# line/Human-Interaction-Generation

Measured on AMD Instinct MI355X. Metric: denoiser-fwd frames/s @ B=64·T=196, higher is better.
Workload: dtype f32; 1 GPU; MotionTransformer forward incl. the per-call cross-attention text side, BASELINE config 2: B=64/GPU T=196 F=150 d=512 L=8 H=8 ff=1024 N=77 Lt=256, linear attention, text embeddings supplied (CLIP stubbed); parallelism=dp1

## Files before the change

human-interaction-generation_amd/csrc/denoiser.hip:

```cpp
#include <stdarg.h>
#include <stdio.h>
#include <string.h>

#include "hig_common.h"
#include "hig_host.h"

static thread_local char g_err[512] = "";
int hig_set_error(int code, const char* fmt, ...) {
  va_list ap;
  va_start(ap, fmt);
  vsnprintf(g_err, sizeof(g_err), fmt, ap);
  va_end(ap);
  return code;
}
extern "C" int hig_last_error(char* buf, int n) {
  if (buf && n > 0) {
    strncpy(buf, g_err, (size_t)n - 1);
    buf[n - 1] = 0;
  }
  return (int)strlen(g_err);
}
extern "C" int hig_version(void) { return 100; }

namespace {
// ... 416 lines not shown
  }
  return &s;
}

thread_local hig_denoiser_plan_t g_last_schedule = {-1};
hig_denoiser_call call_of(int entry, const Dims& D, bool training, bool has_xf_out, int facts, bool capturing) {
  return {entry, D.B, D.T, D.F, D.d, D.E, D.ff, D.L, D.H, D.hd, D.N, D.nsty, D.two, D.full, D.prec, training,
          has_xf_out || entry == HIG_DN_ENTRY_TEXT32 || entry == HIG_DN_ENTRY_TEXT16, facts, capturing};
}
hig_denoiser_plan_t plan_entry(int entry, const Dims& D, bool training, bool has_xf_out, int facts, hipStream_t st, SideStream** side) {
  const hig_denoiser_call c = call_of(entry, D, training, has_xf_out, facts, is_capturing(st));
  hig_denoiser_plan_t p = hig_denoiser_plan_for(c, hig_denoiser_switch_values(), hig_chip_cus(), hig_gemm_wsp32_active());
  SideStream* s = side_streams(p.wants_side_stream, c.capturing);
  if (!s) p.text_fork = p.split = p.fork_emb = p.fork_text = p.wgrad_fork = 0;
  if (side) *side = s;
  g_last_schedule = p;
  return p;
}

struct ThirdStreamJoin {
  hipStream_t s3 = nullptr, st = nullptr;
  hipEvent_t ev = nullptr;
  bool armed = false;
  void arm(hipStream_t s3_, hipEvent_t ev_, hipStream_t st_) { s3 = s3_; ev = ev_; st = st_; armed = true; }
  ~ThirdStreamJoin() {
    if (!armed) return;
    (void)hipEventRecord(ev, s3);
    (void)hipStreamWaitEvent(st, ev, 0);
  }
};

}

static int denoiser_fwd_impl(const hig_dims* dims, const void* const* params, const void* const* derived32, const float* x, const int64_t* t,
                             const int64_t* length, const float* xf_proj, const float* xf_out_for_text, const void* textctx, float* out,
                             void* workspace, int training, hig_stream_t stream);
extern "C" int hig_denoiser_fwd(const hig_dims* dims, const void* const* params, const float* x,
                                const int64_t* t, const int64_t* length, const float* xf_proj,
                                const void* textctx, float* out, void* workspace, int training,
                                hig_stream_t stream) {
  return denoiser_fwd_impl(dims, params, nullptr, x, t, length, xf_proj, nullptr, textctx, out, workspace, training, stream);
}
extern "C" int hig_denoiser_fwd_text(const hig_dims* dims, const void* const* params, const float* x, const int64_t* t,
                                     const int64_t* length, const float* xf_proj, const float* xf_out, void* textctx, float* out,
                                     void* workspace, int training, hig_stream_t stream) {
  HIG_REQUIRE(xf_out, "hig_denoiser_fwd_text: null argument");
  return denoiser_fwd_impl(dims, params, nullptr, x, t, length, xf_proj, xf_out, textctx, out, workspace, training, stream);
}
extern "C" int hig_denoiser_fwd_x(const hig_dims* dims, const void* const* params, const void* const* derived32, const float* x,
                                  const int64_t* t, const int64_t* length, const float* xf_proj, const float* xf_out, void* textctx,
                                  float* out, void* workspace, int training, hig_stream_t stream) {
  return denoiser_fwd_impl(dims, params, derived32, x, t, length, xf_proj, xf_out, textctx, out, workspace, training, stream);
}
static int denoiser_fwd_impl(const hig_dims* dims, const void* const* params, const void* const* derived32, const float* x, const int64_t* t,
                             const int64_t* length, const float* xf_proj, const float* xf_out_for_text, const void* textctx, float* out,
                             void* workspace, int training, hig_stream_t stream) {
  Dims D;
  HIG_TRY(check_dims(dims, D));
  HIG_REQUIRE(params && x && t && xf_proj && textctx && out && workspace, "hig_denoiser_fwd: null argument");
  HIG_REQUIRE(!D.bf16, "hig_denoiser_fwd: bf16 storage goes through hig_denoiser_fwd_bf16");
  const FwdLayout w = fwd_layout(D, training);
  const TextLayout tl = text_layout(D, training);
  float* ws = static_cast<float*>(workspace);
  const float* tc = static_cast<const float*>(textctx);
  hipStream_t st = hig_stream(stream);
  const int d = D.d, E = D.E;
  const int64_t M = D.M;
  const int64_t ss_ld = (int64_t)D.nsty * D.L * 2 * d;
  const int Bp = D.B / 2;

  HIG_TRY(hig_zero_async(ws + w.gtail, HIG_GEMM_TAIL_CNT_BYTES, st));
  const TailScratchScope tail_scope(ws + w.gtail);

  SideStream* side = nullptr;
  const hig_denoiser_plan_t plan = plan_entry(HIG_DN_ENTRY_FWD32, D, training, xf_out_for_text != nullptr,
                                              derived_facts(derived32_table(D, derived32), HIG_D32_TEXT_KV_W), st, &side);
  hipEvent_t* text_ev = nullptr;
  ThirdStreamJoin text_join;
  if (xf_out_for_text) {
    if (plan.text_fork) {
      HIG_TRY(hig_zero_async(ws + w.gtail3, HIG_GEMM_TAIL_CNT_BYTES, st));
      if (hipEventRecord(side->ready, st) != hipSuccess || hipStreamWaitEvent(side->s3, side->ready, 0) != hipSuccess)
        return hig_set_error(HIG_EHIP, "text fork failed");
      hig_gemm_set_tail_scratch(ws + w.gtail3, HIG_GEMM_TAIL_BYTES);
      const int rc = text_context_impl(D, params, derived32, xf_out_for_text, const_cast<void*>(textctx), training, plan.text_batched, side->s3,
                                       side->text_done);
      hig_gemm_set_tail_scratch(ws + w.gtail, HIG_GEMM_TAIL_BYTES);
      text_join.arm(side->s3, side->text_done[0], st);
      if (rc != HIG_OK) return rc;
      text_ev = side->text_done;
    } else {
      HIG_TRY(text_context_impl(D, params, derived32, xf_out_for_text, const_cast<void*>(textctx), training, plan.text_batched, st, nullptr));
    }
  }
  HIG_TRY(hig_timestep_embedding(t, D.B, d, ws + w.te, stream));
  float* few_scratch = ws + w.layer0;
  const int64_t few_floats = w.total - w.layer0;
  HIG_TRY(hig_gemm_few_rows(G(ws + w.te, d, 0, P(params, HIG_P_TE0_W), d, 0, ws + w.te_h, E, D.B, E, d)
                                .epi(HIG_EPI_BIAS, P(params, HIG_P_TE0_B)).prec(D.prec).g, few_scratch, few_floats, st));
  HIG_TRY(hig_gemm_few_rows(G(ws + w.te_h, E, 0, P(params, HIG_P_TE2_W), E, 0, ws + w.emb, E, D.B, E, E)
                                .silu(0).epi(HIG_EPI_BIAS_RES, P(params, HIG_P_TE2_B)).res(xf_proj, E).prec(D.prec).g,
                            few_scratch, few_floats, st));
  HIG_TRY(hig_gemm_few_rows(G(ws + w.emb, E, 0, P(params, HIG_P_STY_EMB_W), E, 0, ws + w.ss, ss_ld, D.B, ss_ld, E)
                                .silu(0).epi(HIG_EPI_BIAS, P(params, HIG_P_STY_EMB_B)).prec(D.prec).g, few_scratch, few_floats,
                            st));
  {
    G ge(x, D.F, 0, P(params, HIG_P_JOINT_W), D.F, 0, ws + w.h0, d, M, d, D.F);
    ge.epi(HIG_EPI_BIAS_POS, P(params, HIG_P_JOINT_B)).pos(P(params, HIG_P_SEQ_EMB), d, D.T).prec(D.prec);
    ge.g.pos_shift = D.two ? 1 : 0;
    HIG_TRY(hig_gemm_launch(ge.g, 1, nullptr, st));
  }
  const int64_t* len_partner = nullptr;
  if (D.two) {
    HIG_TRY(hig_gemm_launch(G(x, (int64_t)D.T * D.F, 0, P(params, HIG_P_JOINT2_W), 4, 0, ws + w.h0, (int64_t)D.T * d,
                              D.B, d, 4).epi(HIG_EPI_BIAS, P(params, HIG_P_JOINT2_B)).g, 1, nullptr, st));
    int64_t* lp = reinterpret_cast<int64_t*>(ws + w.lenp);
    hipLaunchKernelGGL(swap_halves_i64_kernel, dim3((D.B + 255) / 256), dim3(256), 0, st, length, D.B, (int64_t)D.T, lp);
    HIG_CHECK_LAUNCH();
    len_partner = lp;
  }
  const bool fuse_apply = plan.fuse_apply, fold32 = plan.fold32;
  const Derived d32 = derived32_table(D, derived32);
  int layer_rc = HIG_OK;
  auto layer = [&](int l, const float* hin_full, int b0, int nb, hipStream_t s, float* cscr) -> const float* {
    hig_stream_t hs = reinterpret_cast<hig_stream_t>(s);
    float* lb = ws + w.layer0 + w.lstride * l;
    const int64_t r0 = (int64_t)b0 * D.T, Mh = (int64_t)nb * D.T;
    const int64_t aoff = (int64_t)b0 * D.H * D.hd * D.hd;
    const float* ssl = ws + w.ss + (int64_t)(D.nsty * l) * 2 * d + (int64_t)b0 * ss_ld;
    const float* ss_ffn = ssl + (int64_t)(D.nsty - 1) * 2 * d;
    const int64_t* len = length ? length + b0 : nullptr;
    const float* hin = hin_full + r0 * d;
    auto R = [&](int64_t off, int64_t ld) { return lb + off + r0 * ld; };
    auto fail = [&](int rc) -> const float* { layer_rc = rc; return nullptr; };
#define HIG_L(expr) do { const int rc_ = (expr); if (rc_ != HIG_OK) return fail(rc_); } while (0)
    const int np = d >> 6;
    float* lnst = ws + w.lnstats + r0 * np * 2;
    auto folded = [&](int k) { return fold32 && d32.layer(l, HIG_D32_SA_QKV_W + 3 * k) != nullptr; };
// ... 1085 lines not shown
  for (int l = 0; l < D.L; ++l) {
    char* lb = base + tl.layer0 + tl.lstride * l;
    HIG_TRY(hig_ln_bf16(xf_out, 1, D.Lt, D.Mt, D.Lt, PL(params, l, HIG_L_CA_TNORM_W), PL(params, l, HIG_L_CA_TNORM_B), nullptr, 0, 0, 0,
                        lb + tl.xfn, D.Lt, stream));
    HIG_TRY(hig_gemm16_launch(G16(lb + tl.xfn, D.Lt, PL16(params16, l, HIG_L_CA_KV_W), D.Lt, lb + tl.kv, 2 * D.d, D.Mt, 2 * D.d, D.Lt)
                                  .epi(HIG_EPI_BIAS, PL(params, l, HIG_L_CA_KV_B)).g, st));
    HIG_TRY(ctx16(D, plan.ctx_mm16, lb + tl.kv, lb + tl.kv + (int64_t)D.d * 2, 2 * D.d, D.B, D.N, nullptr, reinterpret_cast<float*>(lb + tl.Ac),
                  reinterpret_cast<float*>(lb + tl.kstc), reinterpret_cast<float*>(base + tl.cscr), lb + tl.Atc, stream));
  }
  return HIG_OK;
}

extern "C" int hig_denoiser_fwd_bf16_train(const hig_dims* dims, const void* const* params, const void* const* params16,
                                           const float* x, const int64_t* t, const int64_t* length, const float* xf_proj,
                                           const void* textctx, float* out, void* workspace, hig_stream_t stream) {
  Dims D;
  HIG_TRY(check_dims(dims, D));
  HIG_TRY(require_bf16_train(D, "hig_denoiser_fwd_bf16_train"));
  HIG_REQUIRE(params && params16 && x && t && xf_proj && textctx && out && workspace, "hig_denoiser_fwd_bf16_train: null argument");
  const Fwd16TLayout w = fwd16t_layout(D);
  const Text16TLayout tl = text16t_layout(D);
  char* ws = static_cast<char*>(workspace);
  const char* tc = static_cast<const char*>(textctx);
  hipStream_t st = hig_stream(stream);
  const hig_denoiser_plan_t plan = plan_entry(HIG_DN_ENTRY_FWD16_TRAIN, D, true, false, 0, st);
  const int d = D.d, E = D.E;
  const int64_t M = D.M;
  const int64_t ss_ld = (int64_t)D.nsty * D.L * 2 * d;
  float* te = reinterpret_cast<float*>(ws + w.te);
  float* te_h = reinterpret_cast<float*>(ws + w.te_h);
  float* emb = reinterpret_cast<float*>(ws + w.emb);
  float* ss = reinterpret_cast<float*>(ws + w.ss);
  float* few = reinterpret_cast<float*>(ws + w.few);
  const int64_t few_floats = w.few_bytes / 4;
  HIG_TRY(hig_timestep_embedding(t, D.B, d, te, stream));
  HIG_TRY(hig_gemm_few_rows(G(te, d, 0, P(params, HIG_P_TE0_W), d, 0, te_h, E, D.B, E, d).epi(HIG_EPI_BIAS, P(params, HIG_P_TE0_B)).g,
                            few, few_floats, st));
  HIG_TRY(hig_gemm_few_rows(G(te_h, E, 0, P(params, HIG_P_TE2_W), E, 0, emb, E, D.B, E, E).silu(0)
                                .epi(HIG_EPI_BIAS_RES, P(params, HIG_P_TE2_B)).res(xf_proj, E).g, few, few_floats, st));
  HIG_TRY(hig_gemm_few_rows(G(emb, E, 0, P(params, HIG_P_STY_EMB_W), E, 0, ss, ss_ld, D.B, ss_ld, E).silu(0)
                                .epi(HIG_EPI_BIAS, P(params, HIG_P_STY_EMB_B)).g, few, few_floats, st));
  if (d % 128 == 0 && D.F <= 512) {
    HIG_TRY(hig_joint_embed_bf16(x, M, D.F, P(params, HIG_P_JOINT_W), P(params, HIG_P_JOINT_B), P(params, HIG_P_SEQ_EMB), d, D.T,
                                 D.two ? 1 : 0, ws + w.h0, d, d, few, stream));
  } else {
    float* h32 = few;
    HIG_REQUIRE(M * d * 4 <= w.few_bytes, "hig_denoiser_fwd_bf16_train: d %% 128 != 0 needs M d floats of scratch");
    G ge(x, D.F, 0, P(params, HIG_P_JOINT_W), D.F, 0, h32, d, M, d, D.F);
    ge.epi(HIG_EPI_BIAS_POS, P(params, HIG_P_JOINT_B)).pos(P(params, HIG_P_SEQ_EMB), d, D.T);
    ge.g.pos_shift = D.two ? 1 : 0;
    HIG_TRY(hig_gemm_launch(ge.g, 1, nullptr, st));
    HIG_TRY(hig_cast_bf16(h32, ws + w.h0, M * d, stream));
  }
  const int64_t* len_partner = nullptr;
  const int Bp = D.B / 2;
  if (D.two) {
    float* tok0 = reinterpret_cast<float*>(ws + w.tok0);
    HIG_TRY(hig_gemm_launch(G(x, (int64_t)D.T * D.F, 0, P(params, HIG_P_JOINT2_W), 4, 0, tok0, d, D.B, d, 4)
                                .epi(HIG_EPI_BIAS, P(params, HIG_P_JOINT2_B)).g, 1, nullptr, st));
    hipLaunchKernelGGL(cast_rows_bf16_kernel, dim3((unsigned)(((int64_t)D.B * d + 255) / 256)), dim3(256), 0, st, tok0, (int64_t)d,
                       reinterpret_cast<__bf16*>(ws + w.h0), (int64_t)D.T * d, D.B, d);
    HIG_CHECK_LAUNCH();
    int64_t* lp = reinterpret_cast<int64_t*>(ws + w.lenp);
    hipLaunchKernelGGL(swap_halves_i64_kernel, dim3((D.B + 255) / 256), dim3(256), 0, st, length, D.B, (int64_t)D.T, lp);
    HIG_CHECK_LAUNCH();
    len_partner = lp;
  }
  const void* hin = ws + w.h0;
  for (int l = 0; l < D.L; ++l) {
    char* lb = ws + w.layer0 + w.lstride * l;
    const float* ssl = ss + (int64_t)(D.nsty * l) * 2 * d;
    const bool fuse_front = plan.fuse_front;
    auto sty_out = [&](const void* a, const void* h_in, void* h_out, int out_w, int out_b) -> int {
      return hig_gemm16_launch(G16(a, d, PL16(params16, l, out_w), d, h_out, d, M, d, d).epi(HIG_EPI_BIAS_RES, PL(params, l, out_b)).res16(h_in, d).g, st);
// ... 469 lines not shown
```

human-interaction-generation_amd/csrc/gemm.hip:

```cpp
#include <stdlib.h>

#include "hig_common.h"
#include "hig_host.h"

typedef float f32x16 __attribute__((ext_vector_type(16)));
typedef float f32x4 __attribute__((ext_vector_type(4)));
#ifndef HIG_GEMM_NT
#define HIG_GEMM_NT 0
#endif
#ifndef HIG_GEMM_SETPRIO
#define HIG_GEMM_SETPRIO 1
#endif
#ifndef HIG_GEMM_LDS_EPI
#define HIG_GEMM_LDS_EPI 1
#endif

namespace {

constexpr int BK = 32;
constexpr int NTHREADS = 256;
constexpr int RC_LD = BK + 4;
constexpr int BF_LD = BK + 8;
typedef __bf16 bf16x8 __attribute__((ext_vector_type(8)));
typedef __bf16 bf16x4 __attribute__((ext_vector_type(4)));
// ... 920 lines not shown
    g_tail = TailScratch{nullptr, nullptr, 0};
    return;
  }
  g_tail.cnt = static_cast<unsigned*>(ws);
  g_tail.ws = reinterpret_cast<float*>(static_cast<char*>(ws) + HIG_GEMM_TAIL_CNT_BYTES);
  g_tail.ws_bytes = bytes - HIG_GEMM_TAIL_CNT_BYTES;
}
namespace {
int gemm_dispatch(const hig_gemm_desc& g, int splits, float* slabs, hipStream_t st, const SplitEpilogue& se) {
  const hig_plan p = hig_gemm32_plan(g, g_tail.ws ? g_tail.ws_bytes : 0, hig_gemm_switch_values(), hig_chip_cus());
  if (p.rc != HIG_OK) return hig_set_error(p.rc, "%s", p.msg);
  if (p.launches == 0) return HIG_OK;
  const int64_t slab = (int64_t)g.I * g.J;
  if (splits > 1) HIG_REQUIRE(slabs && g.epi == HIG_EPI_NONE && slab % 4 == 0 && g.ldc == g.J,
                              "hig_gemm: split-R needs slabs, EPI_NONE, dense C");
  if (splits <= 1 && p.path == HIG_GEMM_PATH_WSP32) {
    if (p.launches == 1) return hig_gemm_wsp32_launch(g, p.variant, st);
    hig_gemm_desc p1, p2;
    hig_gemm32_two_pass(g, &p1, &p2);
    HIG_TRY(hig_gemm_wsp32_launch(p1, p.variant, st));
    return hig_gemm_wsp32_launch(p2, HIG_WSP_VARIANT(0, 0), st);
  }
#define CASE(xrs, yrs, xfv, ony, epiv)                                                   \
  if (g.x_rs == xrs && g.y_rs == yrs && g.xf == xfv && (g.xf == HIG_XF_NONE || g.xf_on_y == ony) && \
      g.epi == epiv)                                                                     \
    return launch_sized<xrs, yrs, xfv, ony, epiv>(g, splits, slabs, slab, st, se, p.variant);
  HIG_GEMM32_COMBOS(CASE)
#undef CASE
  return hig_set_error(HIG_EUNSUPPORTED, "hig_gemm: combination x_rs=%d y_rs=%d xf=%d on_y=%d epi=%d not built",
                       g.x_rs, g.y_rs, g.xf, g.xf_on_y, g.epi);
}
}

int hig_gemm_few_rows(const hig_gemm_desc& g, float* scratch, int64_t scratch_floats, hipStream_t st) {
  const int enabled = hig_gemm_switch_values().few_rows_split;
  const int64_t out = (int64_t)g.I * g.J;
  const bool ok = enabled && scratch && g.I > 0 && g.I <= 64 && g.x_rs == 0 && g.y_rs == 0 && g.ldc == g.J && g.J % 4 == 0 &&
                  (g.epi == HIG_EPI_BIAS || g.epi == HIG_EPI_BIAS_RES) && g.bias &&
                  (g.xf == HIG_XF_NONE || g.xf == HIG_XF_SILU) && g.R % 32 == 0 &&
                  (reinterpret_cast<uintptr_t>(g.bias) & 15) == 0 && (reinterpret_cast<uintptr_t>(g.C) & 15) == 0 &&
                  (g.epi != HIG_EPI_BIAS_RES || (g.res && (reinterpret_cast<uintptr_t>(g.res) & 15) == 0 && g.ldr % 4 == 0));
  int splits = 1;
  if (ok) {
    const int64_t tiles = (g.J + 63) / 64;
    int64_t s = 1024 / tiles;
    if (s > g.R / 64) s = g.R / 64;
    if (s > 16) s = 16;
    if (s * out > scratch_floats) s = scratch_floats / out;
    splits = (int)(s < 1 ? 1 : s);
  }
  if (splits <= 1) return hig_gemm_launch(g, 1, nullptr, st);
  hig_gemm_desc p = g;
  p.epi = HIG_EPI_NONE;
  p.bias = nullptr;
  p.res = nullptr;
  return gemm_dispatch(p, splits, scratch, st,
                       SplitEpilogue{g.bias, g.epi == HIG_EPI_BIAS_RES ? g.res : nullptr, g.ldr, g.J / 4});
}

extern "C" int hig_gemm(const hig_gemm_desc* g, hig_stream_t stream) {
  HIG_REQUIRE(g, "hig_gemm: null descriptor");
  HIG_REQUIRE(g->prec == HIG_PREC_F32 || g->prec == HIG_PREC_BF16X3 || g->prec == HIG_PREC_BF16,
              "hig_gemm: unknown prec %d", g->prec);
  return hig_gemm_launch(*g, 1, nullptr, hig_stream(stream));
}

extern "C" int hig_gemm_debug_stamps(void* buf) {
  g_gemm_stamps = static_cast<unsigned long long*>(buf);
  return HIG_OK;
}

extern "C" int64_t hig_gemm_tail_ws_bytes(void) { return HIG_GEMM_TAIL_BYTES; }

static long long g_path_launches[HIG_GEMM_NPATHS];
void hig_gemm_path_count(int path) {
  if (path >= 0 && path < HIG_GEMM_NPATHS) __atomic_fetch_add(&g_path_launches[path], 1, __ATOMIC_RELAXED);
}
extern "C" int64_t hig_gemm_path_launches(int32_t path) {
  if (path < 0 || path >= HIG_GEMM_NPATHS) return -1;
  return __atomic_load_n(&g_path_launches[path], __ATOMIC_RELAXED);
}

extern "C" int hig_gemm_ws(const hig_gemm_desc* g, void* ws, int64_t ws_bytes, hig_stream_t stream) {
  HIG_REQUIRE(g, "hig_gemm_ws: null descriptor");
  HIG_REQUIRE(g->prec == HIG_PREC_F32 || g->prec == HIG_PREC_BF16X3 || g->prec == HIG_PREC_BF16,
              "hig_gemm_ws: unknown prec %d", g->prec);
  HIG_REQUIRE(!ws || (ws_bytes >= HIG_GEMM_TAIL_BYTES && (reinterpret_cast<uintptr_t>(ws) & 15) == 0),
              "hig_gemm_ws: scratch must be 16-byte aligned and hig_gemm_tail_ws_bytes() long");
  hig_gemm_set_tail_scratch(ws, ws_bytes);
// ... 22 lines not shown
```

human-interaction-generation_amd/csrc/gemm_plan.hip:

```cpp
#include <stdarg.h>
#include <stdio.h>

#include "gemm16_epi.h"
#include "hig_host.h"

namespace {

int env_int(const char* v, int dflt) { return v ? atoi(v) : dflt; }

hig_plan served(int path, int variant, int launches = 1) {
  hig_plan p;
  p.rc = HIG_OK; p.path = path; p.launches = launches; p.variant = variant; p.msg[0] = 0;
  return p;
}
hig_plan refused(int rc, const char* fmt, ...) {
  hig_plan p = served(-1, 0, 0);
  p.rc = rc;
  va_list ap;
  va_start(ap, fmt);
  vsnprintf(p.msg, sizeof(p.msg), fmt, ap);
  va_end(ap);
  return p;
}
#define PLAN_REQUIRE(cond, ...) do { if (!(cond)) return refused(HIG_EINVAL, __VA_ARGS__); } while (0)
// ... 96 lines not shown
  if (g.R == 256 ? (folds || g.aux || !(g.epi == HIG_EPI_NONE || g.epi == HIG_EPI_BIAS)) : !(has_bias || has_res || g.epi == HIG_EPI_NONE || g.epi == HIG_EPI_DGELU))
    return -1;
  return HIG_WSP_VARIANT(g.row_stats_out ? 1 : g.row_stats_in ? 2 : 0, g.epi == HIG_EPI_BIAS_GELU && g.aux);
}

int tiled32_tile(const hig_gemm_desc& g, const hig_gemm_switches& sw, int cus) {
  if (g.x_rs) return wgrad_tile(g.I, g.J, g.prec) == 128 ? 0 : 3;
  if (g.row_stats_out || g.row_stats_in) return 3;
  if (sw.tile32 >= 0) return sw.tile32 < 3 ? sw.tile32 : 3;
  auto tiles = [&](int bi, int bj) { return (((int64_t)g.I + bi - 1) / bi) * (((int64_t)g.J + bj - 1) / bj); };
  if (g.prec != HIG_PREC_F32) return tiles(128, 128) >= 300 ? 0 : 3;
  if (tiles(64, 64) > cus) return 3;
  struct Cand { int bi, bj; double ovh; };
  const Cand cands[4] = {{128, 128, 1.00}, {64, 128, 1.02}, {128, 64, 1.03}, {64, 64, 1.04}};
  int best = 0;
  double best_cost = 1e300;
  for (int c = 0; c < 4; ++c) {
    const double cost = (double)((tiles(cands[c].bi, cands[c].bj) + cus - 1) / cus) * cands[c].bi * cands[c].bj * cands[c].ovh;
    if (cost < best_cost) { best_cost = cost; best = c; }
  }
  return best;
}

int tiled32_tail(const hig_gemm_desc& g, int tile, int64_t tail_ws_bytes, const hig_gemm_switches& sw, int cus) {
  const int64_t ntiles = (((int64_t)g.I + 63) / 64) * (((int64_t)g.J + 63) / 64);
  if (!sw.tail32 || tile != 3 || g.x_rs || !hig_gemm32_fast(g) || g.prec != HIG_PREC_F32 || tail_ws_bytes <= 0 || ntiles <= cus || ntiles % cus == 0)
    return 1;
  const int rem = (int)(ntiles % cus), nkt = g.R / 32;
  int s = 1;
  while (2 * s * rem <= cus && nkt % (2 * s) == 0 && nkt / (2 * s) >= 2) s *= 2;
  return (rem <= HIG_GEMM_TAIL_CNT_BYTES / 4 && (int64_t)rem * s * HIG_GEMM_TAIL_UNIT_BYTES <= tail_ws_bytes) ? s : 1;
}

}

const hig_gemm_switches& hig_gemm_switch_values() {
  static const hig_gemm_switches sw = {
      env_int(getenv("HIG_BF16_WSP"), 1),
      env_int(getenv("HIG_BF16_WS"), 1),
      env_int(getenv("HIG_BF16_WS_ROWS"), 2048),
      env_int(getenv("HIG_BF16_WS_NWJ"), 0),
      env_int(getenv("HIG_LNFOLD"), 1),
      env_int(getenv("HIG_LNFOLD1024"), 1),
      env_int(getenv("HIG_BF16_FEWROW"), 1),
      env_int(getenv("HIG_BF16_TILE"), 0),
      env_int(getenv("HIG_F32_WSP"), 1),
      env_int(getenv("HIG_GEMM_TILE"), -1),
      env_int(getenv("HIG_GEMM_TAIL"), 1),
      env_int(getenv("HIG_FEW_ROWS_SPLIT"), 1),
  };
  return sw;
}

bool hig_gemm_wsp32_active() { return hig_gemm_switch_values().wsp32 && ws_chip(hig_chip_cus()); }

hig_plan hig_gemm16_plan(const hig_gemm16_desc& g, const hig_gemm_switches& sw, int cus) {
  PLAN_REQUIRE(g.X && g.Y && g.C, "hig_gemm_bf16: null operand");
  PLAN_REQUIRE(g.I >= 0 && g.J >= 0 && g.R > 0, "hig_gemm_bf16: bad extent");
  if (g.I == 0 || g.J == 0) return served(-1, 0, 0);
  if (g.R % 32 != 0) return refused(HIG_EUNSUPPORTED, "hig_gemm_bf16: the reduce extent must be a multiple of 32 (got %d)", g.R);
  PLAN_REQUIRE(g.ldx % 8 == 0 && g.ldy % 8 == 0 && aligned(g.X, 16) && aligned(g.Y, 16),
               "hig_gemm_bf16: operands must be 16-byte aligned with leading dimensions that are multiples of 8");
  if (epi_has_bias(g.epi)) PLAN_REQUIRE(g.bias, "hig_gemm_bf16: epilogue %d needs a bias", g.epi);
  if (epi_has_res(g.epi)) PLAN_REQUIRE(g.res, "hig_gemm_bf16: epilogue %d needs `res`", g.epi);
  const int wsp = wsp16_variant(g, sw, cus);
  if (wsp >= 0) return served(HIG_GEMM_PATH_WSP16, wsp);
// ... 49 lines not shown
bool hig_gemm_ws16_lnfold_ok(int64_t rows, int d, const hig_gemm_switches& sw, int cus) {
  if (!sw.lnfold || (d == 1024 && !sw.lnfold1024) || rows <= 0 || rows > INT32_MAX || d <= 0 || d > (1 << 20)) return false;
  void* const some = reinterpret_cast<void*>((uintptr_t)4096);
  auto on_fold_kernel = [&](int J, int epi, bool producer) {
    hig_gemm16_desc g;
    memset(&g, 0, sizeof(g));
    g.X = g.Y = g.res = some; g.C = some; g.bias = static_cast<const float*>(some);
    g.ldx = g.ldy = g.ldr = d; g.ldc = J;
    g.I = (int)rows; g.J = J; g.R = d; g.epi = epi;
    if (producer) g.row_stats_out = static_cast<float*>(some);
    else g.row_stats_in = g.ln_colsum = static_cast<const float*>(some);
    const hig_plan p = hig_gemm16_plan(g, sw, cus);
    return p.rc == HIG_OK && (p.path == HIG_GEMM_PATH_WSP16 || p.path == HIG_GEMM_PATH_WS16);
  };
  return on_fold_kernel(d, HIG_EPI_BIAS_RES, true) && on_fold_kernel(3 * d, HIG_EPI_BIAS, false) && on_fold_kernel(d, HIG_EPI_BIAS, false);
}
bool hig_gemm_ws16_lnfold_ok(int64_t rows, int d) { return hig_gemm_ws16_lnfold_ok(rows, d, hig_gemm_switch_values(), hig_chip_cus()); }

static int plan_out(const hig_plan& p, int32_t* path, int32_t* launches, int32_t* variant) {
  if (path) *path = p.path;
  if (launches) *launches = p.launches;
  if (variant) *variant = p.variant;
  return p.rc;
}
extern "C" int hig_gemm_bf16_plan(const hig_gemm16_desc* g, int32_t chip_cus, int32_t* path, int32_t* launches, int32_t* variant) {
  if (!g) return HIG_EINVAL;
  return plan_out(hig_gemm16_plan(*g, hig_gemm_switch_values(), chip_cus > 0 ? chip_cus : hig_chip_cus()), path, launches, variant);
}
extern "C" int hig_gemm_plan(const hig_gemm_desc* g, int32_t has_tail_scratch, int32_t chip_cus, int32_t* path, int32_t* launches, int32_t* variant) {
  if (!g) return HIG_EINVAL;
  return plan_out(hig_gemm32_plan(*g, has_tail_scratch ? HIG_GEMM_TAIL_BYTES - HIG_GEMM_TAIL_CNT_BYTES : 0, hig_gemm_switch_values(),
                                  chip_cus > 0 ? chip_cus : hig_chip_cus()), path, launches, variant);
}
extern "C" int hig_gemm_bf16_lnfold_plan(int64_t rows, int32_t d, int32_t chip_cus) {
  return hig_gemm_ws16_lnfold_ok(rows, d, hig_gemm_switch_values(), chip_cus > 0 ? chip_cus : hig_chip_cus()) ? 1 : 0;
}
```

human-interaction-generation_amd/csrc/hig_host.h:

```cpp
#pragma once
#include <stdlib.h>
#include <string.h>

#include <type_traits>

#include "hig_common.h"

int hig_gemm_launch(const hig_gemm_desc& g, int splits, float* slabs, hipStream_t st);
void hig_gemm_path_count(int path);
void hig_attn_path_count(int path, int split);
int hig_gemm_few_rows(const hig_gemm_desc& g, float* scratch, int64_t scratch_floats, hipStream_t st);

constexpr int64_t HIG_GEMM_TAIL_CNT_BYTES = 1024;
constexpr int64_t HIG_GEMM_TAIL_BYTES = HIG_GEMM_TAIL_CNT_BYTES + 256 * 16384;
void hig_gemm_set_tail_scratch(void* ws, int64_t bytes);

int hig_chip_cus();
inline int hig_chip_xcds() { const int c = hig_chip_cus() / 32; return c < 1 ? 1 : c; }

int hig_gemm16_launch(const hig_gemm16_desc& g, hipStream_t st);
int hig_gemm16_split_launch(const hig_gemm16_desc& g, int splits, float* slabs, int64_t slab_floats, hipStream_t st);
struct hig_wg_reduce {
  const float* slabs; int nsplit; int64_t slab;
  int64_t n4; float* out;
  int64_t nb4; float* dbias;
};
constexpr int HIG_WG_RB_MAX = 12;
int hig_wgrad16_launch(const void* dC, int64_t ldd, const void* act, int64_t ldx, int64_t rows, int J, int K, float* dW, float* dbias,
                       int splits, float* slabs, int64_t slab_floats, hipStream_t st, hig_wg_reduce* deferred = nullptr);
int hig_wgrad16_reduce_batch(const hig_wg_reduce* entries, int n, hipStream_t st);
struct hig_wg_problem {
  const void* dC; int64_t ldd; const void* act; int64_t ldx; int64_t rows; int J, K; float* dW; float* dbias; int splits;
};
constexpr int HIG_WG_GROUP_MAX = 4;
int hig_wgrad16_launch_group(const hig_wg_problem* probs, int n, float* slabs, int64_t slab_floats, hipStream_t st, hig_wg_reduce* deferred,
                             int64_t* used_floats);
int64_t hig_wgrad16_rule_floats(int64_t rows, int J, int K, int64_t room);
int hig_reduce_slabs(const float* slabs, int splits, int64_t slab, int64_t n, float* out, hipStream_t st);
struct hig_gemm_switches {
  int wsp16, ws16, ws_rows, ws_nwj, lnfold, lnfold1024, fewrow16, tile16;
  int wsp32, tile32, tail32;
  int few_rows_split;
};
const hig_gemm_switches& hig_gemm_switch_values();
struct hig_plan { int rc, path, launches, variant; char msg[256]; };
#define HIG_WSP_VARIANT(xt, aux) ((xt) + 4 * ((aux) ? 1 : 0))
#define HIG_WS16_VARIANT(nwj, role) ((nwj) + 256 * (role))
#define HIG_TILE16_VARIANT(rows, bk, ns) ((rows) * 1000 + (bk) * 10 + (ns))
#define HIG_TILE32_VARIANT(tile, tail) ((tile) + 16 * (tail))
hig_plan hig_gemm16_plan(const hig_gemm16_desc& g, const hig_gemm_switches& sw, int cus);
hig_plan hig_gemm32_plan(const hig_gemm_desc& g, int64_t tail_ws_bytes, const hig_gemm_switches& sw, int cus);
bool hig_gemm_ws16_lnfold_ok(int64_t rows, int d);
int hig_gemm_wsp16_launch(const hig_gemm16_desc& g, int variant, hipStream_t st);
int hig_gemm_ws16_launch(const hig_gemm16_desc& g, int variant, hipStream_t st);
int hig_gemm_wsp32_launch(const hig_gemm_desc& g, int variant, hipStream_t st);
constexpr int64_t HIG_GEMM_TAIL_UNIT_BYTES = 256 * 16 * 4;
constexpr int HIG_P32_MAXSEG = 3;
inline int hig_wsp32_segments(int np, int* seg_p0, int* seg_np) {
  int nseg = 0, p0 = 0;
  for (int s = 0; s < HIG_P32_MAXSEG; ++s) { seg_p0[s] = 0; seg_np[s] = 1; }
  while (np > 0) {
    int n = 256;
    while (n > np) n >>= 1;
    if (nseg == HIG_P32_MAXSEG) return -1;
    seg_p0[nseg] = p0; seg_np[nseg] = n; ++nseg;
    p0 += n; np -= n;
  }
  return nseg;
}
inline void hig_gemm32_two_pass(const hig_gemm_desc& g, hig_gemm_desc* p1, hig_gemm_desc* p2) {
  *p1 = g; p1->R = 1024;
  *p2 = g; p2->X = g.X + 1024; p2->Y = g.Y + 1024; p2->R = g.R - 1024;
  p2->epi = HIG_EPI_RES; p2->bias = nullptr; p2->res = g.C; p2->ldr = g.ldc;
}
inline bool hig_gemm32_fast(const hig_gemm_desc& g) {
  auto vec = [](const void* p, int64_t ld) { return ld % 4 == 0 && (reinterpret_cast<uintptr_t>(p) & 15) == 0; };
  return vec(g.X, g.ldx) && vec(g.Y, g.ldy) && g.R % 32 == 0 && g.R > 0 && (!g.x_rs || (g.I % 4 == 0 && g.I >= 4)) && (!g.y_rs || (g.J % 4 == 0 && g.J >= 4));
}
#ifdef HIG_GEMM_PROBE
#define HIG_GEMM32_COMBOS(CASE) CASE(0, 0, HIG_XF_NONE, 0, HIG_EPI_BIAS_GELU)
#else
#define HIG_GEMM32_COMBOS(CASE)                                                                                       \
                                                                                \
  CASE(0, 0, HIG_XF_NONE, 0, HIG_EPI_NONE) CASE(0, 0, HIG_XF_NONE, 0, HIG_EPI_BIAS) CASE(0, 0, HIG_XF_NONE, 0, HIG_EPI_BIAS_GELU) \
  CASE(0, 0, HIG_XF_NONE, 0, HIG_EPI_BIAS_POS) CASE(0, 0, HIG_XF_NONE, 0, HIG_EPI_BIAS_RES)                           \
// ... 225 lines not shown
```

include/hig.h:

```cpp
#ifndef HIG_H
#define HIG_H

#include <stddef.h>
#include <stdint.h>

#ifdef __cplusplus
extern "C" {
#endif

#define HIG_OK 0
#define HIG_EINVAL (-1)
#define HIG_EHIP (-2)
#define HIG_EUNSUPPORTED (-3)

#define HIG_ATTN_LINEAR 0
#define HIG_ATTN_FULL 1

#define HIG_PREC_F32 0
#define HIG_PREC_BF16X3 1
#define HIG_PREC_BF16 2

typedef void* hig_stream_t;

int hig_version(void);
// ... 324 lines not shown
  int32_t I, J, R;
  int32_t epi;
  const float* bias;
  const void* res; int64_t ldr; int32_t res_f32;
  float* row_stats_out;
  const float* row_stats_in;
  const float* ln_colsum;
  void* aux; int64_t ldaux;
} hig_gemm16_desc;
int hig_gemm_bf16(const hig_gemm16_desc* g, hig_stream_t stream);
int64_t hig_gemm_bf16_split_scratch_floats(const hig_gemm16_desc* g, int32_t splits);
int hig_gemm_bf16_split(const hig_gemm16_desc* g, int32_t splits, float* slabs, int64_t slab_floats, hig_stream_t stream);
int hig_gemm_bf16_debug_stamps(void* buf);
int hig_gemm_ws16_debug_stamps(void* buf);
int hig_gemm_wsp16_debug_stamps(void* buf);
int hig_gemm_wsp32_debug_stamps(void* buf);
int64_t hig_gemm_wsp32_launches(void);
#define HIG_GEMM_PATH_TILED32 0
#define HIG_GEMM_PATH_WSP32 1
#define HIG_GEMM_PATH_TAIL32 2
#define HIG_GEMM_PATH_WGRAD_WSP32 3
#define HIG_GEMM_PATH_SPLIT32 4
#define HIG_GEMM_PATH_WSP16 5
#define HIG_GEMM_PATH_WS16 6
#define HIG_GEMM_PATH_FEWROW16 7
#define HIG_GEMM_PATH_TILED16 8
#define HIG_GEMM_PATH_SPLIT16 9
#define HIG_GEMM_PATH_WGRAD16 10
#define HIG_GEMM_NPATHS 11
int64_t hig_gemm_path_launches(int32_t path);
int hig_gemm_bf16_plan(const hig_gemm16_desc* g, int32_t chip_cus, int32_t* path, int32_t* launches, int32_t* variant);
int hig_gemm_plan(const hig_gemm_desc* g, int32_t has_tail_scratch, int32_t chip_cus, int32_t* path, int32_t* launches, int32_t* variant);
int hig_gemm_bf16_lnfold_plan(int64_t rows, int32_t d, int32_t chip_cus);
#define HIG_ATTN_PATH_CTX 0
#define HIG_ATTN_PATH_CTX_MFMA 1
#define HIG_ATTN_PATH_CTX_PART 2
#define HIG_ATTN_PATH_APPLY 3
#define HIG_ATTN_PATH_APPLY_MFMA 4
#define HIG_ATTN_PATH_APPLY_WAVE64 5
#define HIG_ATTN_PATH_APPLY_STY 6
#define HIG_ATTN_PATH_APPLY_STY_WAVE64 7
#define HIG_ATTN_PATH_APPLY_BWD 8
#define HIG_ATTN_PATH_APPLY_BWD_MFMA 9
#define HIG_ATTN_PATH_CTX_BWD 10
#define HIG_ATTN_PATH_CTX_BWD_MFMA 11
#define HIG_ATTN_PATH_FULL_FWD 12
#define HIG_ATTN_PATH_FULL_FWD_MFMA 13
#define HIG_ATTN_PATH_FULL_BWD 14
#define HIG_ATTN_PATH_FULL_BWD_MFMA 15
#define HIG_ATTN_NPATHS 16
int64_t hig_attn_path_launches(int32_t path);
int32_t hig_attn_last_split(void);
#define HIG_ATTN_ENTRY_CTX 0
#define HIG_ATTN_ENTRY_APPLY 1
#define HIG_ATTN_ENTRY_APPLY_STY 2
#define HIG_ATTN_ENTRY_APPLY_BWD 3
#define HIG_ATTN_ENTRY_CTX_BWD 4
#define HIG_ATTN_ENTRY_FULL_FWD 5
#define HIG_ATTN_ENTRY_FULL_BWD 6
#define HIG_ATTN_IO_F32 0
#define HIG_ATTN_IO_BF16 1
#define HIG_ATTN_FACT_IN8 1
#define HIG_ATTN_FACT_IN16 2
#define HIG_ATTN_FACT_OUT8 4
#define HIG_ATTN_FACT_OUT16 8
#define HIG_ATTN_FACT_PAR16 16
// ... 205 lines not shown
```

Baseline: 2.149 million frames/s.

## Add fp32 MFMA few-row GEMM kernel for timestep/style conditioning chain

Adds a dedicated few-row fp32 GEMM kernel that uses 16x16x4 f32 MFMA with the reduction dimension split across eight waves and combined in shared memory. The bias, residual and optional SiLU of the output are applied in the epilogue. The timestep-embedding and style-embedding projections (B=64 rows) route through this kernel instead of split-K GEMM plus a separate reduction. When all three qualify, the SiLU'd output is written to an aux buffer so the next GEMM skips recomputing SiLU on its input. The goal is fewer launches and less slab traffic on a small serial chain, at the cost of a new kernel path with its own shape and alignment constraints.

```diff
diff --git a/human-interaction-generation_amd/csrc/denoiser.hip b/human-interaction-generation_amd/csrc/denoiser.hip
--- a/human-interaction-generation_amd/csrc/denoiser.hip
+++ b/human-interaction-generation_amd/csrc/denoiser.hip
@@ -472,6 +472,25 @@
 
 }
 
+static int conditioning_chain(const void* const* params, const float* te, float* te_h, float* emb, float* ss, const float* xf_proj,
+                              int B, int d, int E, int64_t ss_ld, int prec, float* scratch, int64_t scratch_bytes, hig_stream_t stream) {
+  G te0 = G(te, d, 0, P(params, HIG_P_TE0_W), d, 0, te_h, E, B, E, d).epi(HIG_EPI_BIAS, P(params, HIG_P_TE0_B)).prec(prec);
+  G te2 = G(te_h, E, 0, P(params, HIG_P_TE2_W), E, 0, emb, E, B, E, E).silu(0).epi(HIG_EPI_BIAS_RES, P(params, HIG_P_TE2_B)).res(xf_proj, E).prec(prec);
+  G sty = G(emb, E, 0, P(params, HIG_P_STY_EMB_W), E, 0, ss, ss_ld, B, ss_ld, E).silu(0).epi(HIG_EPI_BIAS, P(params, HIG_P_STY_EMB_B)).prec(prec);
+  const int64_t act = (int64_t)B * E;
+  bool once = scratch && (reinterpret_cast<uintptr_t>(scratch) & 15) == 0 && 2 * act * 4 <= scratch_bytes;
+  for (const G* g : {&te0, &te2, &sty})
+    once = once && hig_gemm_fewrow_plan(g->g, 0, hig_gemm_switch_values(), hig_chip_cus()).form == HIG_FEWROW_FORM_FEWROW32;
+  if (once) {
+    te0.aux(scratch, E);
+    te2.g.X = scratch; te2.g.xf = HIG_XF_NONE; te2.aux(scratch + act, E);
+    sty.g.X = scratch + act; sty.g.xf = HIG_XF_NONE;
+  }
+  HIG_TRY(hig_gemm_fewrow32(&te0.g, scratch, scratch_bytes, stream));
+  HIG_TRY(hig_gemm_fewrow32(&te2.g, scratch, scratch_bytes, stream));
+  return hig_gemm_fewrow32(&sty.g, scratch, scratch_bytes, stream);
+}
+
 static int denoiser_fwd_impl(const hig_dims* dims, const void* const* params, const void* const* derived32, const float* x, const int64_t* t,
                              const int64_t* length, const float* xf_proj, const float* xf_out_for_text, const void* textctx, float* out,
                              void* workspace, int training, hig_stream_t stream);
@@ -534,16 +553,8 @@
     }
   }
   HIG_TRY(hig_timestep_embedding(t, D.B, d, ws + w.te, stream));
-  float* few_scratch = ws + w.layer0;
-  const int64_t few_floats = w.total - w.layer0;
-  HIG_TRY(hig_gemm_few_rows(G(ws + w.te, d, 0, P(params, HIG_P_TE0_W), d, 0, ws + w.te_h, E, D.B, E, d)
-                                .epi(HIG_EPI_BIAS, P(params, HIG_P_TE0_B)).prec(D.prec).g, few_scratch, few_floats, st));
-  HIG_TRY(hig_gemm_few_rows(G(ws + w.te_h, E, 0, P(params, HIG_P_TE2_W), E, 0, ws + w.emb, E, D.B, E, E)
-                                .silu(0).epi(HIG_EPI_BIAS_RES, P(params, HIG_P_TE2_B)).res(xf_proj, E).prec(D.prec).g,
-                            few_scratch, few_floats, st));
-  HIG_TRY(hig_gemm_few_rows(G(ws + w.emb, E, 0, P(params, HIG_P_STY_EMB_W), E, 0, ws + w.ss, ss_ld, D.B, ss_ld, E)
-                                .silu(0).epi(HIG_EPI_BIAS, P(params, HIG_P_STY_EMB_B)).prec(D.prec).g, few_scratch, few_floats,
-                            st));
+  HIG_TRY(conditioning_chain(params, ws + w.te, ws + w.te_h, ws + w.emb, ws + w.ss, xf_proj, D.B, d, E, ss_ld, D.prec, ws + w.layer0,
+                             (w.total - w.layer0) * 4, stream));
   {
     G ge(x, D.F, 0, P(params, HIG_P_JOINT_W), D.F, 0, ws + w.h0, d, M, d, D.F);
     ge.epi(HIG_EPI_BIAS_POS, P(params, HIG_P_JOINT_B)).pos(P(params, HIG_P_SEQ_EMB), d, D.T).prec(D.prec);
@@ -1695,14 +1706,8 @@
   float* emb = reinterpret_cast<float*>(ws + w.emb);
   float* ss = reinterpret_cast<float*>(ws + w.ss);
   float* few = reinterpret_cast<float*>(ws + w.few);
-  const int64_t few_floats = w.few_bytes / 4;
   HIG_TRY(hig_timestep_embedding(t, D.B, d, te, stream));
-  HIG_TRY(hig_gemm_few_rows(G(te, d, 0, P(params, HIG_P_TE0_W), d, 0, te_h, E, D.B, E, d).epi(HIG_EPI_BIAS, P(params, HIG_P_TE0_B)).g,
-                            few, few_floats, st));
-  HIG_TRY(hig_gemm_few_rows(G(te_h, E, 0, P(params, HIG_P_TE2_W), E, 0, emb, E, D.B, E, E).silu(0)
-                                .epi(HIG_EPI_BIAS_RES, P(params, HIG_P_TE2_B)).res(xf_proj, E).g, few, few_floats, st));
-  HIG_TRY(hig_gemm_few_rows(G(emb, E, 0, P(params, HIG_P_STY_EMB_W), E, 0, ss, ss_ld, D.B, ss_ld, E).silu(0)
-                                .epi(HIG_EPI_BIAS, P(params, HIG_P_STY_EMB_B)).g, few, few_floats, st));
+  HIG_TRY(conditioning_chain(params, te, te_h, emb, ss, xf_proj, D.B, d, E, ss_ld, HIG_PREC_F32, few, w.few_bytes, stream));
   if (d % 128 == 0 && D.F <= 512) {
     HIG_TRY(hig_joint_embed_bf16(x, M, D.F, P(params, HIG_P_JOINT_W), P(params, HIG_P_JOINT_B), P(params, HIG_P_SEQ_EMB), d, D.T,
                                  D.two ? 1 : 0, ws + w.h0, d, d, few, stream));
diff --git a/human-interaction-generation_amd/csrc/gemm.hip b/human-interaction-generation_amd/csrc/gemm.hip
--- a/human-interaction-generation_amd/csrc/gemm.hip
+++ b/human-interaction-generation_amd/csrc/gemm.hip
@@ -976,29 +976,22 @@
 }
 }
 
-int hig_gemm_few_rows(const hig_gemm_desc& g, float* scratch, int64_t scratch_floats, hipStream_t st) {
-  const int enabled = hig_gemm_switch_values().few_rows_split;
-  const int64_t out = (int64_t)g.I * g.J;
-  const bool ok = enabled && scratch && g.I > 0 && g.I <= 64 && g.x_rs == 0 && g.y_rs == 0 && g.ldc == g.J && g.J % 4 == 0 &&
-                  (g.epi == HIG_EPI_BIAS || g.epi == HIG_EPI_BIAS_RES) && g.bias &&
-                  (g.xf == HIG_XF_NONE || g.xf == HIG_XF_SILU) && g.R % 32 == 0 &&
-                  (reinterpret_cast<uintptr_t>(g.bias) & 15) == 0 && (reinterpret_cast<uintptr_t>(g.C) & 15) == 0 &&
-                  (g.epi != HIG_EPI_BIAS_RES || (g.res && (reinterpret_cast<uintptr_t>(g.res) & 15) == 0 && g.ldr % 4 == 0));
-  int splits = 1;
-  if (ok) {
-    const int64_t tiles = (g.J + 63) / 64;
-    int64_t s = 1024 / tiles;
-    if (s > g.R / 64) s = g.R / 64;
-    if (s > 16) s = 16;
-    if (s * out > scratch_floats) s = scratch_floats / out;
-    splits = (int)(s < 1 ? 1 : s);
-  }
-  if (splits <= 1) return hig_gemm_launch(g, 1, nullptr, st);
-  hig_gemm_desc p = g;
-  p.epi = HIG_EPI_NONE;
-  p.bias = nullptr;
-  p.res = nullptr;
-  return gemm_dispatch(p, splits, scratch, st,
+extern "C" int hig_gemm_fewrow32(const hig_gemm_desc* gp, void* scratch, int64_t scratch_bytes, hig_stream_t stream) {
+  HIG_REQUIRE(gp, "hig_gemm_fewrow32: null descriptor");
+  HIG_REQUIRE(gp->prec == HIG_PREC_F32 || gp->prec == HIG_PREC_BF16X3 || gp->prec == HIG_PREC_BF16,
+              "hig_gemm_fewrow32: unknown prec %d", gp->prec);
+  const hig_gemm_desc& g = *gp;
+  hipStream_t st = hig_stream(stream);
+  const bool has_scratch = scratch && scratch_bytes > 0 && (reinterpret_cast<uintptr_t>(scratch) & 15) == 0;
+  const hig_fewrow_plan_t p = hig_gemm_fewrow_plan(g, has_scratch ? scratch_bytes / 4 : 0, hig_gemm_switch_values(), hig_chip_cus());
+  if (p.form == HIG_FEWROW_FORM_FEWROW32) return hig_gemm_fewrow32_launch(g, p.col_units, st);
+  if (g.aux) return hig_set_error(HIG_EUNSUPPORTED, "hig_gemm_fewrow32: `aux` (silu of the output) on a call gemm_fewrow32 does not serve");
+  if (p.form == HIG_FEWROW_FORM_PLAIN) return hig_gemm_launch(g, 1, nullptr, st);
+  hig_gemm_desc q = g;
+  q.epi = HIG_EPI_NONE;
+  q.bias = nullptr;
+  q.res = nullptr;
+  return gemm_dispatch(q, p.splits, static_cast<float*>(scratch), st,
                        SplitEpilogue{g.bias, g.epi == HIG_EPI_BIAS_RES ? g.res : nullptr, g.ldr, g.J / 4});
 }
 
diff --git a/human-interaction-generation_amd/csrc/gemm_fewrow32.hip b/human-interaction-generation_amd/csrc/gemm_fewrow32.hip
--- /dev/null
+++ b/human-interaction-generation_amd/csrc/gemm_fewrow32.hip
@@ -0,0 +1,151 @@
+#include <hip/hip_runtime.h>
+
+#include "hig_host.h"
+
+namespace {
+
+typedef float f32x4 __attribute__((ext_vector_type(4)));
+
+constexpr int FR_WAVES = 8;
+constexpr int FR_THREADS = 64 * FR_WAVES;
+constexpr int FR_SLICE = 16;
+constexpr int FR_STAGE = FR_SLICE * FR_WAVES;
+
+long long g_fr_launches = 0;
+
+struct FrArgs {
+  const float* X; const float* W; float* C; const float* bias; const float* res; float* aux;
+  int64_t ldx, ldy, ldr, ldaux;
+  int I, J, R, silu;
+};
+
+__device__ __forceinline__ f32x4 fr_load(const float* p) { return *reinterpret_cast<const f32x4*>(p); }
+
+template <int NU, int NB, int D>
+__global__ __launch_bounds__(FR_THREADS) void gemm_fewrow32_kernel(FrArgs a) {
+  __shared__ f32x4 part[2][FR_WAVES][NB][64];
+  const int lane = threadIdx.x & 63, wave = __builtin_amdgcn_readfirstlane(threadIdx.x >> 6);
+  const int li = lane & 15, g = lane >> 4;
+  const int64_t j0 = (int64_t)blockIdx.x * (16 * NU);
+  const int lrow = lane >> 2, lchunk = lane & 3;
+  const int perm = 4 * (4 * li + g);
+  const float* wp = a.W + (j0 + lrow) * a.ldy + 4 * lchunk;
+  const float* xp[NB];
+#pragma unroll
+  for (int ib = 0; ib < NB; ++ib) xp[ib] = a.X + (int64_t)min(16 * ib + lrow, a.I - 1) * a.ldx + 4 * lchunk;
+  auto to_fragment = [&](float v) { return __int_as_float(__builtin_amdgcn_ds_bpermute(perm, __float_as_int(v))); };
+  const int64_t unit_stride = 16 * a.ldy;
+
+  f32x4 acc[NU][NB];
+#pragma unroll
+  for (int u = 0; u < NU; ++u)
+#pragma unroll
+    for (int ib = 0; ib < NB; ++ib) acc[u][ib] = f32x4{0.f, 0.f, 0.f, 0.f};
+
+  f32x4 wb[D][NU], xb[D][NB];
+  const int nstage = (a.R + FR_STAGE - 1) / FR_STAGE;
+  auto slice = [&](int k) { return min(k, nstage - 1) * FR_STAGE + wave * FR_SLICE; };
+  auto fetch = [&](int k, f32x4* w, f32x4* x) {
+    const int r = min(slice(k), a.R - FR_SLICE);
+#pragma unroll
+    for (int u = 0; u < NU; ++u) w[u] = fr_load(wp + u * unit_stride + r);
+#pragma unroll
+    for (int ib = 0; ib < NB; ++ib) x[ib] = fr_load(xp[ib] + r);
+  };
+  auto multiply = [&](int k, f32x4* w, f32x4* x) {
+    if (k >= nstage || slice(k) >= a.R) return;
+    auto prepare = [&](int c) {
+#pragma unroll
+      for (int ib = 0; ib < NB; ++ib) x[ib][c] = to_fragment(x[ib][c]);
+#pragma unroll
+      for (int u = 0; u < NU; ++u) w[u][c] = to_fragment(w[u][c]);
+      if (a.silu) {
+#pragma unroll
+        for (int ib = 0; ib < NB; ++ib) x[ib][c] = hig_silu(x[ib][c]);
+      }
+      __builtin_amdgcn_sched_barrier(0);
+    };
+    prepare(0);
+#pragma unroll
+    for (int c = 0; c < 4; ++c) {
+      if (c < 3) prepare(c + 1);
+#pragma unroll
+      for (int u = 0; u < NU; ++u)
+#pragma unroll
+        for (int ib = 0; ib < NB; ++ib) acc[u][ib] = __builtin_amdgcn_mfma_f32_16x16x4f32(w[u][c], x[ib][c], acc[u][ib], 0, 0, 0);
+      __builtin_amdgcn_sched_barrier(0);
+    }
+  };
+
+#pragma unroll
+  for (int d = 0; d < D; ++d) fetch(d, wb[d], xb[d]);
+  for (int s0 = 0; s0 < nstage; s0 += D) {
+#pragma unroll
+    for (int d = 0; d < D; ++d) {
+      multiply(s0 + d, wb[d], xb[d]);
+      fetch(s0 + d + D, wb[d], xb[d]);
+    }
+  }
+
+#pragma unroll
+  for (int u = 0; u < NU; ++u) {
+#pragma unroll
+    for (int ib = 0; ib < NB; ++ib) part[u & 1][wave][ib][lane] = acc[u][ib];
+    __syncthreads();
+    if (wave < NB) {
+      f32x4 s = part[u & 1][0][wave][lane];
+#pragma unroll
+      for (int w = 1; w < FR_WAVES; ++w) s += part[u & 1][w][wave][lane];
+      const int i = 16 * wave + li;
+      const int64_t j = j0 + 16 * u + 4 * g;
+      s += fr_load(a.bias + j);
+      if (i < a.I) {
+        if (a.res) s += fr_load(a.res + i * a.ldr + j);
+        *reinterpret_cast<f32x4*>(a.C + (int64_t)i * a.J + j) = s;
+        if (a.aux) *reinterpret_cast<f32x4*>(a.aux + i * a.ldaux + j) = f32x4{hig_silu(s[0]), hig_silu(s[1]), hig_silu(s[2]), hig_silu(s[3])};
+      }
+    }
+  }
+}
+
+template <int NU, int D>
+void launch(const FrArgs& a, hipStream_t st) {
+  const dim3 grid(a.J / (16 * NU)), block(FR_THREADS);
+  switch ((a.I + 15) / 16) {
+    case 1: hipLaunchKernelGGL((gemm_fewrow32_kernel<NU, 1, D>), grid, block, 0, st, a); break;
+    case 2: hipLaunchKernelGGL((gemm_fewrow32_kernel<NU, 2, D>), grid, block, 0, st, a); break;
+    case 3: hipLaunchKernelGGL((gemm_fewrow32_kernel<NU, 3, D>), grid, block, 0, st, a); break;
+    default: hipLaunchKernelGGL((gemm_fewrow32_kernel<NU, 4, D>), grid, block, 0, st, a); break;
+  }
+}
+
+}
+
+int hig_gemm_fewrow32_launch(const hig_gemm_desc& g, int col_units, hipStream_t st) {
+  auto al16 = [](const void* p) { return p && (reinterpret_cast<uintptr_t>(p) & 15) == 0; };
+  HIG_REQUIRE(g.prec == HIG_PREC_F32 && g.I >= 1 && g.I <= 64 && !g.x_rs && !g.y_rs && g.R >= 64 && g.R % 64 == 0 && g.J >= 16 &&
+                  g.J % 16 == 0 && g.ldc == g.J && (g.xf == HIG_XF_NONE || (g.xf == HIG_XF_SILU && !g.xf_on_y)) &&
+                  (g.epi == HIG_EPI_BIAS || g.epi == HIG_EPI_BIAS_RES) && al16(g.X) && al16(g.Y) && al16(g.C) && al16(g.bias) &&
+                  g.ldx % 4 == 0 && g.ldy % 4 == 0 && g.ldx >= g.R && g.ldy >= g.R &&
+                  (g.epi != HIG_EPI_BIAS_RES || (al16(g.res) && g.ldr % 4 == 0 && g.ldr >= g.J)) &&
+                  (!g.aux || (al16(g.aux) && g.ldaux % 4 == 0 && g.ldaux >= g.J)),
+              "hig_gemm_fewrow32: a call the few-row fp32 kernel does not serve");
+  HIG_REQUIRE(col_units >= 1 && (g.J / 16) % col_units == 0, "hig_gemm_fewrow32: %d column units do not divide J / 16 = %d", col_units, g.J / 16);
+  FrArgs a;
+  a.X = g.X; a.W = g.Y; a.C = g.C; a.bias = g.bias; a.res = g.epi == HIG_EPI_BIAS_RES ? g.res : nullptr;
+  a.aux = g.aux; a.ldx = g.ldx; a.ldy = g.ldy; a.ldr = g.ldr; a.ldaux = g.ldaux;
+  a.I = g.I; a.J = g.J; a.R = g.R; a.silu = g.xf == HIG_XF_SILU;
+  switch (col_units) {
+    case 6: launch<6, 2>(a, st); break;
+    case 4: launch<4, 3>(a, st); break;
+    case 3: launch<3, 3>(a, st); break;
+    case 2: launch<2, 4>(a, st); break;
+    case 1: launch<1, 6>(a, st); break;
+    default: return hig_set_error(HIG_EINVAL, "hig_gemm_fewrow32: no instance with %d column units", col_units);
+  }
+  HIG_CHECK_LAUNCH();
+  __atomic_fetch_add(&g_fr_launches, 1, __ATOMIC_RELAXED);
+  return HIG_OK;
+}
+
+extern "C" int64_t hig_gemm_fewrow32_launches(void) { return __atomic_load_n(&g_fr_launches, __ATOMIC_RELAXED); }
diff --git a/human-interaction-generation_amd/csrc/gemm_plan.hip b/human-interaction-generation_amd/csrc/gemm_plan.hip
--- a/human-interaction-generation_amd/csrc/gemm_plan.hip
+++ b/human-interaction-generation_amd/csrc/gemm_plan.hip
@@ -152,6 +152,57 @@
   return (rem <= HIG_GEMM_TAIL_CNT_BYTES / 4 && (int64_t)rem * s * HIG_GEMM_TAIL_UNIT_BYTES <= tail_ws_bytes) ? s : 1;
 }
 
+bool fewrow32_serves(const hig_gemm_desc& g) {
+  auto rows = [](const void* p, int64_t ld, int64_t extent) { return p && aligned(p, 16) && ld % 4 == 0 && ld >= extent; };
+  if (g.prec != HIG_PREC_F32 || g.I < 1 || g.I > 64 || g.x_rs || g.y_rs) return false;
+  if (g.R < 64 || g.R % 64 != 0 || g.J < 16 || g.J % 16 != 0 || g.ldc != g.J) return false;
+  if (!(g.xf == HIG_XF_NONE || (g.xf == HIG_XF_SILU && !g.xf_on_y))) return false;
+  if (!(g.epi == HIG_EPI_BIAS || g.epi == HIG_EPI_BIAS_RES) || !g.bias || !aligned(g.bias, 16)) return false;
+  if (g.xcolsum || g.row_stats_out || g.row_stats_in) return false;
+  if (!rows(g.X, g.ldx, g.R) || !rows(g.Y, g.ldy, g.R) || !g.C || !aligned(g.C, 16)) return false;
+  if (g.aux && !rows(g.aux, g.ldaux, g.J)) return false;
+  return g.epi != HIG_EPI_BIAS_RES || rows(g.res, g.ldr, g.J);
+}
+int fewrow32_units(int J, int cus) {
+  const int units = J / 16, cands[5] = {6, 4, 3, 2, 1};
+  int best = 1;
+  double best_cost = 1e300;
+  for (int nu : cands) {
+    if (units % nu != 0) continue;
+    const double cost = (double)(((int64_t)units / nu + cus - 1) / cus) * (nu + 0.5);
+    if (cost < best_cost) { best_cost = cost; best = nu; }
+  }
+  return best;
+}
+int fewrow_splits(const hig_gemm_desc& g, int64_t scratch_floats) {
+  const int64_t out = (int64_t)g.I * g.J;
+  const bool ok = scratch_floats > 0 && g.I > 0 && g.I <= 64 && g.x_rs == 0 && g.y_rs == 0 && g.ldc == g.J && g.J > 0 && g.J % 4 == 0 && g.R > 0 &&
+                  (g.epi == HIG_EPI_BIAS || g.epi == HIG_EPI_BIAS_RES) && g.bias &&
+                  (g.xf == HIG_XF_NONE || g.xf == HIG_XF_SILU) && g.R % 32 == 0 && aligned(g.bias, 16) && aligned(g.C, 16) &&
+                  (g.epi != HIG_EPI_BIAS_RES || (g.res && aligned(g.res, 16) && g.ldr % 4 == 0));
+  if (!ok) return 1;
+  const int64_t tiles = ((int64_t)g.J + 63) / 64;
+  int64_t s = 1024 / tiles;
+  if (s > g.R / 64) s = g.R / 64;
+  if (s > 16) s = 16;
+  if (s * out > scratch_floats) s = scratch_floats / out;
+  return (int)(s < 1 ? 1 : s);
+}
+
+}
+
+hig_fewrow_plan_t hig_gemm_fewrow_plan(const hig_gemm_desc& g, int64_t scratch_floats, const hig_gemm_switches& sw, int cus) {
+  hig_fewrow_plan_t p = {HIG_FEWROW_FORM_PLAIN, 1, 0, 0};
+  if (!sw.few_rows_split) return p;
+  if (cus > 0 && fewrow32_serves(g)) {
+    p.form = HIG_FEWROW_FORM_FEWROW32;
+    p.col_units = fewrow32_units(g.J, cus);
+    p.blocks = g.J / 16 / p.col_units;
+    return p;
+  }
+  const int s = fewrow_splits(g, scratch_floats);
+  if (s > 1) { p.form = HIG_FEWROW_FORM_SPLIT; p.splits = s; }
+  return p;
 }
 
 const hig_gemm_switches& hig_gemm_switch_values() {
@@ -267,6 +318,17 @@
   return plan_out(hig_gemm32_plan(*g, has_tail_scratch ? HIG_GEMM_TAIL_BYTES - HIG_GEMM_TAIL_CNT_BYTES : 0, hig_gemm_switch_values(),
                                   chip_cus > 0 ? chip_cus : hig_chip_cus()), path, launches, variant);
 }
+extern "C" int hig_gemm_fewrow32_plan(const hig_gemm_desc* g, int64_t scratch_bytes, int32_t chip_cus, int32_t* form, int32_t* splits,
+                                      int32_t* col_units, int32_t* blocks) {
+  if (!g) return HIG_EINVAL;
+  const hig_fewrow_plan_t p = hig_gemm_fewrow_plan(*g, scratch_bytes > 0 ? scratch_bytes / 4 : 0, hig_gemm_switch_values(),
+                                                   chip_cus > 0 ? chip_cus : hig_chip_cus());
+  if (form) *form = p.form;
+  if (splits) *splits = p.splits;
+  if (col_units) *col_units = p.col_units;
+  if (blocks) *blocks = p.blocks;
+  return HIG_OK;
+}
 extern "C" int hig_gemm_bf16_lnfold_plan(int64_t rows, int32_t d, int32_t chip_cus) {
   return hig_gemm_ws16_lnfold_ok(rows, d, hig_gemm_switch_values(), chip_cus > 0 ? chip_cus : hig_chip_cus()) ? 1 : 0;
 }
diff --git a/human-interaction-generation_amd/csrc/hig_host.h b/human-interaction-generation_amd/csrc/hig_host.h
--- a/human-interaction-generation_amd/csrc/hig_host.h
+++ b/human-interaction-generation_amd/csrc/hig_host.h
@@ -9,7 +9,6 @@
 int hig_gemm_launch(const hig_gemm_desc& g, int splits, float* slabs, hipStream_t st);
 void hig_gemm_path_count(int path);
 void hig_attn_path_count(int path, int split);
-int hig_gemm_few_rows(const hig_gemm_desc& g, float* scratch, int64_t scratch_floats, hipStream_t st);
 
 constexpr int64_t HIG_GEMM_TAIL_CNT_BYTES = 1024;
 constexpr int64_t HIG_GEMM_TAIL_BYTES = HIG_GEMM_TAIL_CNT_BYTES + 256 * 16384;
@@ -51,6 +50,9 @@
 hig_plan hig_gemm16_plan(const hig_gemm16_desc& g, const hig_gemm_switches& sw, int cus);
 hig_plan hig_gemm32_plan(const hig_gemm_desc& g, int64_t tail_ws_bytes, const hig_gemm_switches& sw, int cus);
 bool hig_gemm_ws16_lnfold_ok(int64_t rows, int d);
+struct hig_fewrow_plan_t { int form, splits, col_units, blocks; };
+hig_fewrow_plan_t hig_gemm_fewrow_plan(const hig_gemm_desc& g, int64_t scratch_floats, const hig_gemm_switches& sw, int cus);
+int hig_gemm_fewrow32_launch(const hig_gemm_desc& g, int col_units, hipStream_t st);
 int hig_gemm_wsp16_launch(const hig_gemm16_desc& g, int variant, hipStream_t st);
 int hig_gemm_ws16_launch(const hig_gemm16_desc& g, int variant, hipStream_t st);
 int hig_gemm_wsp32_launch(const hig_gemm_desc& g, int variant, hipStream_t st);
diff --git a/include/hig.h b/include/hig.h
--- a/include/hig.h
+++ b/include/hig.h
@@ -380,6 +380,13 @@
 int hig_gemm_bf16_plan(const hig_gemm16_desc* g, int32_t chip_cus, int32_t* path, int32_t* launches, int32_t* variant);
 int hig_gemm_plan(const hig_gemm_desc* g, int32_t has_tail_scratch, int32_t chip_cus, int32_t* path, int32_t* launches, int32_t* variant);
 int hig_gemm_bf16_lnfold_plan(int64_t rows, int32_t d, int32_t chip_cus);
+#define HIG_FEWROW_FORM_PLAIN 0
+#define HIG_FEWROW_FORM_SPLIT 1
+#define HIG_FEWROW_FORM_FEWROW32 2
+int hig_gemm_fewrow32(const hig_gemm_desc* g, void* scratch, int64_t scratch_bytes, hig_stream_t stream);
+int hig_gemm_fewrow32_plan(const hig_gemm_desc* g, int64_t scratch_bytes, int32_t chip_cus, int32_t* form, int32_t* splits,
+                           int32_t* col_units, int32_t* blocks);
+int64_t hig_gemm_fewrow32_launches(void);
 #define HIG_ATTN_PATH_CTX 0
 #define HIG_ATTN_PATH_CTX_MFMA 1
 #define HIG_ATTN_PATH_CTX_PART 2
```

Result: no change. 2.154 million frames/s (median of 6 runs) (+0.3%).
